# etiiiR/pixel-nerf

Hardware: AMD Instinct MI355X
Metric: rays/sec (coarse+fine, 64+64 samples) (higher is better)
Workload: dtype f32 (f16x3)

## Files before the change

include/pnr_abi.h:

```cpp
#ifndef PNR_ABI_H
#define PNR_ABI_H

#include <stddef.h>
#include <stdint.h>

#ifdef __cplusplus
extern "C" {
#endif

#define PNR_ABI_VERSION 8

typedef enum pnr_status {
    PNR_OK = 0,
    PNR_ERR_INVALID = -1,
    PNR_ERR_UNSUPPORTED = -2,
    PNR_ERR_HIP = -3,
    PNR_ERR_WORKSPACE = -4
} pnr_status;

typedef void *pnr_stream_t;

typedef struct pnr_scene {
    const float *latent;
    const float *cams;
// ... 106 lines not shown

int pnr_point_query_proj(const pnr_scene *scene, const pnr_mlp_desc *desc, const void *packed,
                         const float *proj, const float *xyz, const float *viewdirs,
                         int64_t points_per_obj, float *out, void *workspace,
                         size_t workspace_bytes, pnr_stream_t stream);
int pnr_render_forward_proj(const pnr_scene *scene, const pnr_mlp_desc *desc,
                            const void *coarse_packed, const void *fine_packed,
                            const float *coarse_proj, const float *fine_proj,
                            const pnr_rays *rays, const pnr_rng *rng,
                            const pnr_render_cfg *cfg, const pnr_render_out *out,
                            void *workspace, size_t workspace_bytes, pnr_stream_t stream,
                            void *const *events);

int32_t pnr_render_set_fused(int32_t on);

int pnr_sample_coarse(const float *rays, int64_t n_rays, int32_t n_coarse,
                      const float *u_coarse, int32_t lindisp, float *z,
                      pnr_stream_t stream);

int pnr_sample_fine(const float *rays, int64_t n_rays, int32_t n_coarse,
                    const float *z_coarse, const float *coarse_weights,
                    const float *coarse_depth, int32_t n_fine, int32_t n_fine_depth,
                    float depth_std, const float *u_fine, const float *u_fine_jit,
                    const float *n_depth, int32_t lindisp, float *z_fine,
                    pnr_stream_t stream);

int pnr_composite(const float *z, const float *raw, const float *rays, int64_t n_rays,
                  int32_t k, int32_t white_bkgd, float *weights, float *rgb, float *depth,
                  pnr_stream_t stream);

// ... 109 lines not shown
```

pixel-nerf_amd/csrc/abi.cpp:

```cpp
#include <atomic>
#include <cstdarg>
#include <cstdio>
#include <cstring>

#include "march_dev.h"
#include "pnr_launch.h"

namespace pnr {

static thread_local char g_err[1024];
static std::atomic<int> g_fused_default{2};

void set_error(const char *fmt, ...) {
    va_list ap;
    va_start(ap, fmt);
    vsnprintf(g_err, sizeof(g_err), fmt, ap);
    va_end(ap);
}

int fail(int status, const char *fmt, ...) {
    va_list ap;
    va_start(ap, fmt);
    vsnprintf(g_err, sizeof(g_err), fmt, ap);
    va_end(ap);
// ... 447 lines not shown
                                   nullptr, nullptr, 1, n * kf, raw_new, xsum, st, nullptr, fine_proj)))
            return rc;
        if ((rc = launch_merge_raw(origin, rawc, raw_new, n, kc, kf, rawf, st))) return rc;
    } else if ((rc = launch_point_mlp(*scene, *desc, fine_packed, rays->rays, zf, kall, rays->rays_per_obj,
                                      nullptr, nullptr, 1, n * kall, rawf, xsum, st, nullptr, fine_proj))) {
        return rc;
    }
    if ((rc = mark(5))) return rc;
    if ((rc = launch_composite(zf, rawf, rays->rays, n, kall, cfg->white_bkgd, out->fine_weights,
                               out->fine_rgb, out->fine_depth, st)))
        return rc;
    return mark(6);
}

int32_t pnr_render_set_fused(int32_t on) { return g_fused_default.exchange(on < 0 || on > 3 ? 2 : on); }

int pnr_sample_coarse(const float *rays, int64_t n_rays, int32_t n_coarse, const float *u_coarse,
                      int32_t lindisp, float *z, pnr_stream_t stream) {
    if (n_rays < 0 || n_coarse < 1) return fail(PNR_ERR_INVALID, "pnr_sample_coarse: bad sizes");
    if (n_rays > 0 && (!rays || !u_coarse || !z)) return fail(PNR_ERR_INVALID, "pnr_sample_coarse: NULL");
    return launch_sample_coarse(rays, n_rays, n_coarse, RngSrc{u_coarse, 0, 0, PNR_RNG_U_COARSE}, lindisp, z,
                                (hipStream_t)stream);
}

int pnr_sample_fine(const float *rays, int64_t n_rays, int32_t n_coarse, const float *z_coarse,
                    const float *coarse_weights, const float *coarse_depth, int32_t n_fine,
                    int32_t n_fine_depth, float depth_std, const float *u_fine,
                    const float *u_fine_jit, const float *n_depth, int32_t lindisp, float *z_fine,
                    pnr_stream_t stream) {
    if (n_rays < 0 || n_coarse < 1 || n_fine < 1 || n_fine_depth < 0 || n_fine_depth > n_fine)
// ... 133 lines not shown
```

pixel-nerf_amd/csrc/march_dev.h:

```cpp
#pragma once
#include "pnr_common.h"

namespace pnr {

#ifndef EPI_T
#define EPI_DECL
#define EPI_T(i) ((void)0)
#endif

__device__ __forceinline__ void wave_lds_sync() { asm volatile("s_waitcnt lgkmcnt(0)" ::: "memory"); }

__device__ __forceinline__ float linspace_at(int i, int n, float end, float step) {
    if (n == 1) return 0.0f;
    return (i < n / 2) ? mul_rn(step, (float)i) : sub_rn(end, mul_rn(step, (float)(n - 1 - i)));
}

__device__ __forceinline__ float coarse_z(const RngSrc &u, int64_t b, int kc, int k, float near, float far,
                                          bool lindisp) {
    const float end = (float)(1.0 - 1.0 / (double)kc);
    const float lstep = (kc > 1) ? __fdiv_rn(end, (float)(kc - 1)) : 0.0f;
    const float step = (float)(1.0 / (double)kc);
    const float t = add_rn(linspace_at(k, kc, end, lstep), mul_rn(rng_uniform(u, b, kc, k), step));
    return t_to_z(t, near, far, lindisp);
}

template <int S>
__device__ __forceinline__ float composite_wave(int lane, int64_t b, int K, float far, const float (&zk)[S],
                                                const f4 (&v)[S], int white_bkgd, float *weights,
                                                float *rgb_out, float *depth_out, float (&wk)[S]) {
    double carry = 1.0;
    float sr = 0.f, sg = 0.f, sb = 0.f, sd = 0.f, sw = 0.f;
#pragma unroll
    for (int i = 0; i < S; ++i) {
        const int k = 64 * i + lane;
        const bool valid = k < K;
        const float nxt0 = i + 1 < S ? __int_as_float(__builtin_amdgcn_readlane(__float_as_int(zk[i + 1 < S ? i + 1 : i]), 0))
                                     : far;
        const float zl = dpp_f<0x130>(nxt0, zk[i]);
// ... 217 lines not shown
```

pixel-nerf_amd/csrc/mlp.hip:

```cpp
#include "pnr_diag.h"
#include <cstddef>

#ifdef PNR_EPI_TIMING
__device__ unsigned long long g_epi[8];
#endif

#include "march_dev.h"
#include "mlp_dev.h"
#include "pnr_launch.h"

namespace pnr {
namespace mlpk {

#ifdef PNR_PHASE_TIMING
__device__ unsigned long long g_phase[PT_SLOTS];
#endif

struct Args {
    const float *packed;
    Layout L;
    int render_mode;
    const float *rays, *zs;
    int K;
    int64_t rays_per_obj;
// ... 56 lines not shown
        float *w = scr;
#pragma unroll
        for (int i = 0; i < S; ++i) w[64 * i + lane] = wk[i];
        wave_lds_sync();
        sample_fine_wave(lane, b, near, far, COLS * S, w, buf, depth, kf, c->kfd, c->depth_std, RngSrc{}, RngSrc{},
                         RngSrc{}, c->lindisp != 0, c->n_sort, scr + 128, scr + 256, nullptr, c->z_fine, nullptr,
                         nullptr, true, d, c->single ? const_cast<float *>(buf) : nullptr);
    }
}
__device__ __forceinline__ void march_epilogue(const Args &a, int64_t b, const float *buf, const float *nf,
                                               float *scr, int lane, bool fine_pass) {
    if ((fine_pass ? march_cfg(a)->kpt_f : march_cfg(a)->kpt) == 1) march_ray<1>(a, b, buf, nf, scr, lane, fine_pass);
    else march_ray<2>(a, b, buf, nf, scr, lane, fine_pass);
}

template <int PREC, bool PZ, bool MARCH>
__global__ __launch_bounds__(NTHR) void k_point_mlp(Args a) {
    constexpr int KD = H_DIST;
    constexpr bool HP = is_h(PREC);
    constexpr int NP = nparts(PREC);
    static_assert(PREC != 1 || PZ, "PREC 1 is built for the projected-latent path only");
    extern __shared__ __attribute__((aligned(16))) float smem[];
    constexpr FwdLds M = fwd_lds(HP);
    float *inbuf = smem;
    const int tid = threadIdx.x;
    const int lane = tid & 63;
    const int wave = __builtin_amdgcn_readfirstlane(tid >> 6);
    const int g = lane >> 4;
    const int cl = lane & 15;
    const Layout &L = a.L;

    const int64_t wl_off = (int64_t)(RTW * wave) * 256 + lane * 4;
// ... 29 lines not shown
#ifdef PNR_PHASE_TIMING
    for (int i = 0; i < PT_SLOTS; ++i) gc.pt[i] = 0;
    gc.pt_last = __builtin_amdgcn_s_memtime();
#endif
    constexpr int FPT = 64 / WAVES;

    const int64_t P = a.n_points, PS = P * a.ns;
    float *sv_f = a.save, *sv_z = a.save ? a.save + PS * 64 : nullptr;
    auto sv_slot = [&](int i) { return sv_z + PS * H * (1 + i); };
    uint32_t *sv_mask = a.save ? reinterpret_cast<uint32_t *>(a.save + save_mask_offset(L.n_blocks, PS)) : nullptr;
    auto pre_publish_sync = [&]() {
        if constexpr (!HP)
            lds_barrier();
    };
    auto publish_relu = [&](const Acc &acc, int64_t tile, int save_idx, int64_t row0) {
        if (a.save) {
            save_relu(acc, sv_slot(save_idx) + row0 * H, tile, P, wave, lane);
            save_mask(acc, sv_mask + PS * 16 * save_idx + row0 * 16, tile, P, wave, lane);
        }
        if constexpr (HP) {
            PT(gc, 17);
            relu_colmax(acc, cmax, wave, lane);
            PT(gc, 13);
            lds_barrier();
            PT(gc, 14);
            relu_store_split<true, NP>(acc, P0, P1, cmax, ecol, wave, lane, gc.ecl);
            PT(gc, 15);
        } else {
            store_relu(acc, inbuf, wave, lane);
        }
    };

    Acc x, h;
    int *s_next = reinterpret_cast<int *>(inbuf + M.s_next);
    float *hpart = inbuf + M.hpart;
    float *mreg = inbuf + M.mreg;
    float *mscr = inbuf + M.mscr;
    float *mnf = inbuf + M.mnf;
    const int kpt = MARCH ? march_cfg(a)->kpt : 1;
    const bool single = MARCH && march_cfg(a)->single;
    const int upt = single ? kpt + march_cfg(a)->kpt_f : kpt;
    float *petab_f = inbuf + M.petab_f;
    if (single && wave == 1) petab_f[lane & 31] = march_cfg(a)->packed_f[lane & 31];
    auto grab = [&]() -> int {
        const int64_t T = a.n_tiles / upt;
        const int x0 = blockIdx.x & 7;
        for (int k = 0; k < 8; ++k) {
            const int x = (x0 + k) & 7;
            const int64_t lo = x * T / 8, hi = (x + 1) * T / 8;
            if (lo >= hi) continue;
            const int64_t i = lo + claim_one(a.tile_ctr + 16 * x);
            if (i < hi) return (int)(i * upt);
        }
        return (int)a.n_tiles;
    };
    if (wave == 0) *s_next = grab();
    lds_barrier();
    for (int64_t tile = *s_next; tile < a.n_tiles; tile = *s_next) {
        const int64_t unit = tile / upt;
        const int s_in = (int)(tile - unit * upt);
        const bool pass_f = single && s_in >= kpt;
        const int sub = pass_f ? s_in - kpt : s_in;
        const int kpt_t = pass_f ? march_cfg(a)->kpt_f : kpt;
        auto ray_of = [&]() -> int64_t {
            const int *o = MARCH ? march_cfg(a)->order : nullptr;
            if (!o) return unit;
            const int64_t r = o[unit];
            return r >= 0 && r < a.n_tiles / upt ? r : unit;
        };
        auto PK = [&]() -> const float * { return pass_f ? march_cfg(a)->packed_f : a.packed; };
        auto PJ_ = [&]() -> const float * { return pass_f ? march_cfg(a)->proj_f : a.proj; };
        const float *bias = PK() + L.off_bias;
        gc.hdr = PK();
        auto xp_ptr = [&]() { return a.xsum + (int64_t)blockIdx.x * (2 * COLS * H) + wave * (RTW * CT * 256) + opaque_lane(lane) * 4; };
        auto xs_ptr = [&]() { return xp_ptr() + COLS * H; };

        for (int v = 0; v < a.ns; ++v) {
            const int tid_t = opaque_lane(tid);
            const int col = tid_t / WAVES, qt = tid_t % WAVES;
            const int64_t p_raw = tile * COLS + col;
            const int64_t p = p_raw < a.n_points ? p_raw : a.n_points - 1;
            float px, py, pz, dx, dy, dz, zz = 0.f;
            int64_t obj;
            if (a.render_mode) {
                const int64_t b = MARCH ? ray_of() : p / a.K;
                const int kk = MARCH ? sub * COLS + col : (int)(p - b * a.K);
                const int kt = MARCH ? COLS * kpt_t : a.K;
                const float *ray = a.rays + b * 8;
                if (MARCH && pass_f) {
                    lds_barrier();
                    zz = mreg[kk];
                } else if (MARCH && march_cfg(a)->sample_coarse) {
                    const CfgPtr m = march_cfg(a);
                    zz = coarse_z(ld_rng(m->u_coarse), b, kt, kk, ray[6], ray[7], m->lindisp != 0);
                    float *zo = m->z_out;
                    if (zo && qt == 0 && v == 0) zo[b * kt + kk] = zz;
                } else {
                    zz = a.zs[b * kt + kk];
                }
                dx = ray[3]; dy = ray[4]; dz = ray[5];
                px = add_rn(ray[0], mul_rn(zz, dx));
                py = add_rn(ray[1], mul_rn(zz, dy));
                pz = add_rn(ray[2], mul_rn(zz, dz));
                obj = b / a.rays_per_obj;
            } else {
                px = a.xyz[p * 3 + 0]; py = a.xyz[p * 3 + 1]; pz = a.xyz[p * 3 + 2];
                if (a.dirs) { dx = a.dirs[p * 3 + 0]; dy = a.dirs[p * 3 + 1]; dz = a.dirs[p * 3 + 2]; }
                else { dx = dy = dz = 0.f; }
                obj = p / a.points_per_obj;
            }
            PT_WAIT();
            PT(gc, 8);
            const float *cam = a.cams + (obj * a.ns + v) * 16;
            float xr[3], vd[3], xc[3];
#pragma unroll
            for (int i = 0; i < 3; ++i) {
                const float r0 = cam[3 * i], r1 = cam[3 * i + 1], r2 = cam[3 * i + 2];
                xr[i] = add_rn(add_rn(mul_rn(r0, px), mul_rn(r1, py)), mul_rn(r2, pz));
                vd[i] = add_rn(add_rn(mul_rn(r0, dx), mul_rn(r1, dy)), mul_rn(r2, dz));
                xc[i] = add_rn(xr[i], cam[9 + i]);
            }
            const float fx = cam[12], fy = cam[13], cx = cam[14], cy = cam[15];
            PT_WAIT();
            PT(gc, 9);
            lds_barrier();
            PT(gc, 10);
            if (MARCH && qt == 0 && v == 0) {
                if (!pass_f) mreg[sub * COLS + col] = zz;
                if (col == 0 && sub == 0) {
                    const float *rr = a.rays + ray_of() * 8;
                    mnf[0] = rr[6];
                    mnf[1] = rr[7];
                }
            }
            {
                const int npe = 3 * L.pe_n;
                const float *pet = MARCH && pass_f ? petab_f : petab;
                float fv[FPT];
#pragma unroll
                for (int i = 0; i < FPT; ++i) {
                    const int f = FPT * qt + i;
                    float val = 0.f;
                    if (f < 3) val = xr[f];
                    else if (f < 3 + npe) {
                        const int m = f - 3, q = m / 3, d = m - 3 * q;
                        const float xd = d == 0 ? xr[0] : (d == 1 ? xr[1] : xr[2]);
                        val = sinf(add_rn(pet[16 + q], mul_rn(xd, pet[q])));
                    } else if (f < 6 + npe) {
                        const int d = f - 3 - npe;
                        val = d == 0 ? vd[0] : (d == 1 ? vd[1] : vd[2]);
                    }
                    fv[i] = val;
                }
                if (a.save && p_raw < a.n_points) {
#pragma unroll
                    for (int i = 0; i < FPT / 4; ++i)
                        *reinterpret_cast<f4 *>(sv_f + (v * P + p_raw) * 64 + FPT * qt + 4 * i) =
                            f4{fv[4 * i], fv[4 * i + 1], fv[4 * i + 2], fv[4 * i + 3]};
                }
                if constexpr (HP) {
                    float m = 0.f;
#pragma unroll
                    for (int i = 0; i < FPT; ++i) m = fmaxf(m, fabsf(fv[i]));
#pragma unroll
                    for (int o = 1; o < WAVES; o <<= 1) m = fmaxf(m, __shfl_xor(m, o, 64));
                    const int e = scale_exp(m);
                    const float sc = __builtin_ldexpf(1.f, e);
#pragma unroll
                    for (int i = 0; i < FPT / 4; ++i)
                        put_split4(P0, P1, col * ROWH + swz(col, FPT * qt + 4 * i),
                                   f4{fv[4 * i], fv[4 * i + 1], fv[4 * i + 2], fv[4 * i + 3]}, sc);
                    if (qt == 0) ecol[col] = e;
                } else {
#pragma unroll
                    for (int i = 0; i < FPT / 4; ++i)
                        *reinterpret_cast<f4 *>(inbuf + col * LDS_LD + FPT * qt + 4 * i) =
                            f4{fv[4 * i], fv[4 * i + 1], fv[4 * i + 2], fv[4 * i + 3]};
                }
            }
            PT(gc, 11);
            float u = mul_rn(__fdiv_rn(-xc[0], xc[2]), fx);
            float w = mul_rn(__fdiv_rn(-xc[1], xc[2]), fy);
            u = add_rn(u, cx);
            w = add_rn(w, cy);
            const float wlf = (float)a.wl, hlf = (float)a.hl;
            const float lsx = mul_rn(__fdiv_rn(wlf, sub_rn(wlf, 1.f)), 2.f);
            const float lsy = mul_rn(__fdiv_rn(hlf, sub_rn(hlf, 1.f)), 2.f);
            const float gx = sub_rn(mul_rn(u, __fdiv_rn(lsx, a.img_w)), 1.f);
            const float gy = sub_rn(mul_rn(w, __fdiv_rn(lsy, a.img_h)), 1.f);
            float ix = mul_rn(add_rn(gx, 1.f), mul_rn(sub_rn(wlf, 1.f), 0.5f));
            float iy = mul_rn(add_rn(gy, 1.f), mul_rn(sub_rn(hlf, 1.f), 0.5f));
            ix = fminf(fmaxf(ix, 0.f), wlf - 1.f);
            iy = fminf(fmaxf(iy, 0.f), hlf - 1.f);
            const float x0f = floorf(ix), y0f = floorf(iy);
            const float we = sub_rn(ix, x0f), wn = sub_rn(iy, y0f);
            const float ee = sub_rn(1.f, we), ss = sub_rn(1.f, wn);
            float wnw = mul_rn(ss, ee), wne = mul_rn(ss, we), wsw = mul_rn(wn, ee), wse = mul_rn(wn, we);
            const int x0 = (int)x0f, y0 = (int)y0f;
            const int x1 = x0 + 1 < a.wl ? x0 + 1 : x0, y1 = y0 + 1 < a.hl ? y0 + 1 : y0;
            if (x0 + 1 >= a.wl) { wne = 0.f; wse = 0.f; }
            if (y0 + 1 >= a.hl) { wsw = 0.f; wse = 0.f; }
            if (qt == 0) {
                const uint32_t base = (uint32_t)((obj * a.ns + v) * (int64_t)a.hl * a.wl * H);
                const uint32_t o00 = base + (uint32_t)(y0 * a.wl + x0) * H, o01 = base + (uint32_t)(y0 * a.wl + x1) * H;
                const uint32_t o10 = base + (uint32_t)(y1 * a.wl + x0) * H, o11 = base + (uint32_t)(y1 * a.wl + x1) * H;
                float *t = gtab + col * 8;
                *reinterpret_cast<f4 *>(t) = f4{__uint_as_float(o00), __uint_as_float(o01),
                                                __uint_as_float(o10), __uint_as_float(o11)};
                *reinterpret_cast<f4 *>(t + 4) = f4{wnw, wne, wsw, wse};
            }
            PT(gc, 12);
            lds_barrier();
            PT(gc, 0);
            add_bias(x, bias, wave, lane, false);
            layer_gemm<PREC, NKB_IN, KD, false, 2>(x, PK() + L.off_lin_in, gc, 0);
            for (int blk = 0; blk < L.ncomb; ++blk) {
                const int lz = layer_index(blk, 0, L.ncomb);
                if constexpr (PZ) {
// ... 62 lines not shown
                layer_gemm<PREC, NKB, KD, HP>(h, PK() + L.off_l512 + (int64_t)(lz + 1) * L.layer_floats, gc, 2 + lz,
                                          HP ? &R0 : nullptr);
                pre_publish_sync();
                HRing<KD, NP> R1;
                const float *w1p = PK() + L.off_l512 + (int64_t)(lz + 2) * L.layer_floats;
                if constexpr (HP) hring_prime(R1, w1p + opaque_lane((int)gc.ws_off));
                f4 nb1[RTW];
                load_bias(nb1, bias + (3 + lz) * H, wave, lane);
                publish_relu(h, tile, L.n_blocks + blk, v * P);
                lds_barrier();
                PT(gc, 16);
                set_bias(x, nb1, true);
                layer_gemm<PREC, NKB, KD, HP>(x, PK() + L.off_l512 + (int64_t)(lz + 2) * L.layer_floats, gc, 3 + lz,
                                          HP ? &R1 : nullptr);
            }
            if (a.ns > 1) {
                float *xs = xs_ptr();
                if (v == 0) {
#pragma unroll
                    for (int r = 0; r < RTW; ++r)
#pragma unroll
                        for (int c = 0; c < CT; ++c)
                            *reinterpret_cast<f4 *>(xs + (r * CT + c) * 256) = x[r][c];
                } else if (v < a.ns - 1) {
#pragma unroll
                    for (int r = 0; r < RTW; ++r)
#pragma unroll
                        for (int c = 0; c < CT; ++c) {
                            f4 *ptr = reinterpret_cast<f4 *>(xs + (r * CT + c) * 256);
                            *ptr = *ptr + x[r][c];
                        }
// ... 27 lines not shown
            HRing<KD, NP> R1;
            const float *w1p = PK() + L.off_l512 + (int64_t)(l0 + 1) * L.layer_floats;
            if constexpr (HP) hring_prime(R1, w1p + opaque_lane((int)gc.ws_off));
            f4 nb1[RTW];
            load_bias(nb1, bias + (2 + l0) * H, wave, lane);
            publish_relu(h, tile, L.n_blocks + blk, 0);
            lds_barrier();
            PT(gc, 16);
            set_bias(x, nb1, true);
            layer_gemm<PREC, NKB, KD, HP>(x, PK() + L.off_l512 + (int64_t)(l0 + 1) * L.layer_floats, gc, 2 + l0,
                                      HP ? &R1 : nullptr);
        }
        if (wave == 0) *s_next = s_in + 1 < upt ? (int)tile + 1 : grab();
        pre_publish_sync();
        if constexpr (HP) {
            if (a.save) {
                save_relu(x, sv_slot(2 * L.n_blocks), tile, P, wave, lane);
                save_mask(x, sv_mask + PS * 16 * (2 * L.n_blocks), tile, P, wave, lane);
            }
        } else {
            publish_relu(x, tile, 2 * L.n_blocks, 0);
            lds_barrier();
        }
        PT(gc, 16);
        PT(gc, 3);
        if (HP) {
            const int ln = opaque_lane(lane), g4 = ln >> 4, c16 = ln & 15;
            const float *w32 = PK() + L.off_out32;
            f4 o[CT];
#pragma unroll
            for (int c = 0; c < CT; ++c) o[c] = f4{0.f, 0.f, 0.f, 0.f};
#pragma unroll
            for (int r = 0; r < RTW; ++r) {
// ... 92 lines not shown
    if (reset) {
        static const unsigned long long zero[mlpk::PT_SLOTS] = {};
        if (hipMemcpyToSymbol(HIP_SYMBOL(mlpk::g_phase), zero, sizeof(zero)) != hipSuccess) return -1;
    }
    return 0;
}
#endif
int64_t mlp_save_floats(const pnr_mlp_desc &d, int64_t n_points) {
    return mlpk::save_floats_per_point(d.n_blocks) * n_points;
}

size_t mlp_xsum_bytes(int ns) {
    (void)ns;
    return sizeof(float) * (size_t)device_cu_count() * 2 * mlpk::COLS * mlpk::H + 512;
}

int launch_point_mlp(const pnr_scene &sc, const pnr_mlp_desc &d, const void *packed,
                     const float *rays, const float *zs, int K, int64_t rays_per_obj,
                     const float *xyz, const float *dirs, int64_t points_per_obj,
                     int64_t n_points, float *out, float *xsum_ws, hipStream_t st, float *save,
                     const float *proj, const MarchCfg *march) {
    if (n_points == 0) return PNR_OK;
    if (d.precision == PNR_PREC_F16 && (!proj || save))
        return fail(PNR_ERR_UNSUPPORTED, "precision 1 (f16) is inference only on the projected-latent path: it "
                    "needs the latent projection and takes no activation save; use precision 3 (f16x3)");
    if (proj && save) return fail(PNR_ERR_UNSUPPORTED, "the activation save (training) needs the latent gather path");
    if (march && (!rays || save || (march->kpt != 1 && march->kpt != 2) || K != mlpk::COLS * march->kpt ||
                  n_points % K != 0 || (march->kf > 0 && (K > 64 || march->n_sort > 128 || K + march->kf > march->n_sort))))
        return fail(PNR_ERR_INVALID, "point_mlp: fused march needs K = 64 kpt (kpt 1 or 2) and kc + kf <= 128");
    if (march && march->single &&
// ... 13 lines not shown
    a.ns = sc.n_views; a.hl = sc.latent_h; a.wl = sc.latent_w;
    a.img_w = sc.image_w; a.img_h = sc.image_h;
    a.out = out;
    a.xsum = xsum_ws;
    a.march = march != nullptr;
    if (march) a.m = *march;
    a.n_tiles = (n_points + mlpk::COLS - 1) / mlpk::COLS;
    a.save = save;
    a.proj = proj;
    a.proj_stride = (int64_t)sc.n_obj * sc.n_views * sc.latent_h * sc.latent_w * mlpk::H;
    const int cus = device_cu_count();
    if (a.n_tiles >= (1ll << 31)) return fail(PNR_ERR_UNSUPPORTED, "more than 2^31 point tiles in one launch");
    a.tile_ctr = reinterpret_cast<int *>(xsum_ws + (size_t)cus * 2 * mlpk::COLS * mlpk::H);
    if (hipMemsetAsync(a.tile_ctr, 0, 512, st) != hipSuccess) return fail(PNR_ERR_HIP, "point_mlp: hipMemsetAsync failed");
    const int64_t grid = a.n_tiles < cus ? a.n_tiles : cus;
    const size_t lds = mlpk::lds_bytes(mlpk::fwd_lds(mlpk::is_h(d.precision)), march != nullptr);
#define PNR_LAUNCH_MLP(P)                                                                              \
    do {                                                                                               \
        if (proj && march) hipLaunchKernelGGL((mlpk::k_point_mlp<P, true, true>), dim3((unsigned)grid), dim3(mlpk::NTHR), lds, st, a); \
        else if (proj) hipLaunchKernelGGL((mlpk::k_point_mlp<P, true, false>), dim3((unsigned)grid), dim3(mlpk::NTHR), lds, st, a); \
        else if (march) hipLaunchKernelGGL((mlpk::k_point_mlp<P, false, true>), dim3((unsigned)grid), dim3(mlpk::NTHR), lds, st, a); \
        else hipLaunchKernelGGL((mlpk::k_point_mlp<P, false, false>), dim3((unsigned)grid), dim3(mlpk::NTHR), lds, st, a);     \
    } while (0)
    switch (d.precision) {
    case PNR_PREC_F16:
        if (march) hipLaunchKernelGGL((mlpk::k_point_mlp<1, true, true>), dim3((unsigned)grid), dim3(mlpk::NTHR), lds, st, a);
        else hipLaunchKernelGGL((mlpk::k_point_mlp<1, true, false>), dim3((unsigned)grid), dim3(mlpk::NTHR), lds, st, a);
        break;
    case PNR_PREC_F16X3: PNR_LAUNCH_MLP(3); break;
    case PNR_PREC_BF16X6: PNR_LAUNCH_MLP(6); break;
    case PNR_PREC_BF16X9: PNR_LAUNCH_MLP(9); break;
// ... 8 lines not shown
```

pixel-nerf_amd/csrc/mlp_layout.h:

```cpp
#pragma once
#include "pnr_common.h"

namespace pnr {
namespace mlpk {

constexpr int H = 512;
constexpr int NRT = H / 16;
constexpr int NKB = H / 16;
constexpr int NKB_IN = 4;
constexpr int WAVES = 8;
constexpr int NTHR = 64 * WAVES;
constexpr int RTW = NRT / WAVES;
constexpr int CT = 4;
constexpr int COLS = 16 * CT;
constexpr int LDS_LD = H + 4;
constexpr int KB_FLOATS = NRT * 256;
constexpr int LAYER_FLOATS = NKB * KB_FLOATS;
constexpr int HDR = 64;
constexpr int KS32 = H / 32;
constexpr int KS32_IN = 2;
constexpr int SRT_FLOATS = 768;
constexpr int SKS_FLOATS = NRT * SRT_FLOATS;
constexpr int SRT16_FLOATS = 512;
constexpr int SKS16_FLOATS = NRT * SRT16_FLOATS;
// ... 46 lines not shown

__host__ __device__ constexpr int64_t save_floats_per_point(int n_blocks) {
    return 64 + (int64_t)H * (2 + 2 * n_blocks) + 16 * (2 * n_blocks + 1);
}
__host__ __device__ constexpr int64_t save_mask_offset(int n_blocks, int64_t n_points) {
    return (64 + (int64_t)H * (2 + 2 * n_blocks)) * n_points;
}

__device__ __forceinline__ int scale_exp(float m) {
    if (!(m > 0.f) || !(m < 3.0e38f)) return 0;
    int e = 14 - __builtin_amdgcn_frexp_expf(m);
    return e < -64 ? -64 : (e > 40 ? 40 : e);
}

struct FwdLds {
    int stg, gtab, cmax, ecol, petab, s_next, prog, hpart, mreg, mscr, mnf, petab_f, end;
};
constexpr int IMG_H_FLOATS = PART_HALVES;
constexpr int MARCH_BUF_FLOATS = 640;
constexpr FwdLds fwd_lds(bool hp) {
    FwdLds m = {};
    m.stg = COLS * LDS_LD;
    m.gtab = hp ? IMG_H_FLOATS : m.stg + 2 * STG_FLOATS;
    m.cmax = m.gtab + COLS * 8;
    m.ecol = m.cmax + COLS * 8;
    m.petab = hp ? m.ecol + COLS : m.gtab + COLS * 8;
    m.s_next = m.petab + 32;
    m.prog = m.petab + 40;
    m.hpart = m.petab + 64;
    m.mreg = hp ? m.hpart + WAVES * COLS * 4 : m.petab + 36;
    m.mscr = m.mreg + MARCH_BUF_FLOATS;
    m.mnf = m.mscr + 3 * 128;
    m.petab_f = m.mnf + 4;
    m.end = m.petab_f + 32;
    return m;
}
constexpr size_t lds_bytes(const FwdLds &m, bool march) { return sizeof(float) * (size_t)(march ? m.end : m.mreg); }
constexpr int MARCH_LDS_FLOATS = fwd_lds(true).end - fwd_lds(true).mreg;

struct BwdLds {
    int cmax, ecol, prog, end;
};
constexpr BwdLds bwd_lds() {
    BwdLds m = {};
    m.cmax = IMG_H_FLOATS;
    m.ecol = m.cmax + COLS * 8;
    m.prog = m.ecol + COLS;
    m.end = m.prog + WAVES;
    return m;
}
constexpr size_t lds_bytes(const BwdLds &m) { return sizeof(float) * (size_t)m.end; }

static_assert(lds_bytes(fwd_lds(true), false) == 147968 && lds_bytes(fwd_lds(false), false) == 158864 &&
              lds_bytes(bwd_lds()) == 137504, "LDS totals");
static_assert(lds_bytes(fwd_lds(true), true) == 147968 + 4 * MARCH_LDS_FLOATS &&
              lds_bytes(fwd_lds(false), true) == 158864 + 4 * MARCH_LDS_FLOATS &&
              fwd_lds(false).end - fwd_lds(false).mreg == MARCH_LDS_FLOATS, "LDS totals with the march region");
static_assert(lds_bytes(fwd_lds(true), true) <= 160 * 1024 && lds_bytes(fwd_lds(false), true) <= 160 * 1024 &&
              lds_bytes(bwd_lds()) <= 160 * 1024, "one workgroup's LDS");
static_assert(sizeof(float) * COLS * LDS_LD <= 2 * sizeof(_Float16) * PART_HALVES,
              "the fp32 stage fits in the split image it aliases");

}
}
```

pixel-nerf_amd/csrc/pnr_launch.h:

```cpp
#pragma once
#include "pnr_common.h"

namespace pnr {

struct MarchCfg;

int launch_sample_coarse(const float *, int64_t, int, const RngSrc &, int, float *, hipStream_t);
int launch_sample_fine(const float *, int64_t, int, const float *, const float *, const float *,
                       int, int, float, const RngSrc &, const RngSrc &, const RngSrc &, int, float *,
                       hipStream_t, int *origin = nullptr, float *z_new = nullptr);
int launch_rng_fill(const RngSrc &, int64_t, int, float *, hipStream_t);
int launch_merge_raw(const int *, const float *, const float *, int64_t, int, int, float *, hipStream_t);
int launch_gen_rays(const float *, int64_t, int, int, int, float, float, float, float, float, float,
                    float *, hipStream_t);
int launch_composite(const float *, const float *, const float *, int64_t, int, int, float *,
                     float *, float *, hipStream_t);
int sort_width(int n);
size_t mlp_packed_bytes(const pnr_mlp_desc &);
int mlp_check_desc(const pnr_mlp_desc &);
int mlp_pack(const pnr_mlp_weights &, void *, size_t, hipStream_t);
size_t mlp_packed_t_bytes(const pnr_mlp_desc &);
int mlp_pack_t(const pnr_mlp_weights &, const void *, void *, size_t, hipStream_t);
size_t mlp_xsum_bytes(int ns);
int64_t mlp_save_floats(const pnr_mlp_desc &d, int64_t n_points);
int launch_point_mlp(const pnr_scene &, const pnr_mlp_desc &, const void *, const float *,
                     const float *, int, int64_t, const float *, const float *, int64_t, int64_t,
                     float *, float *, hipStream_t, float *save = nullptr, const float *proj = nullptr,
                     const MarchCfg *march = nullptr);
int launch_mlp_bwd(const pnr_mlp_desc &, const void *, const void *, const float *, const float *, const float *,
                   int64_t, float *, float *, hipStream_t, float *, void *, size_t, int n_views);
size_t mlp_bwd_workspace_bytes(const pnr_mlp_desc &, int64_t);
size_t wgrad_workspace_bytes(int, int64_t);
int launch_wgrad(const float *const *, const float *const *, float *const *, int, int64_t, void *, size_t,
                 hipStream_t, int arith);
int launch_fold_bn(const pnr_bn_fold *, int, int64_t, hipStream_t);
int launch_latent_cl_bwd(const float *, float *const *, const int32_t *, const int32_t *, const int32_t *, int, int, int,
                         int, hipStream_t);
int launch_latent_cl(const float *const *, const int32_t *, const int32_t *, const int32_t *, int, int, float *,
                     int, int, bool, hipStream_t);
int launch_composite_bwd(const float *, const float *, const float *, int64_t, int, int, const float *,
                         const float *, const float *, float *, float *, hipStream_t);
int launch_points_in_bwd(const float *, const float *, int, int64_t, int64_t, int, const float *, const float *,
                         int, int, float, float, const float *, int, const float *, const float *, float *,
// ... 14 lines not shown
```

pixel-nerf_amd/csrc/torch_ops.cpp:

```cpp
#include <ATen/ATen.h>
#include <c10/core/DeviceGuard.h>
#include <c10/hip/HIPStream.h>
#include <torch/library.h>

#include <vector>

#include "../../include/pnr_abi.h"

namespace {

void check(int rc, const char *what) {
    TORCH_CHECK(rc == PNR_OK, what, " failed (status ", rc, "): ", pnr_last_error());
}

void *stream_of(const at::Tensor &t) {
    return c10::hip::getCurrentHIPStream(t.device().index()).stream();
}

const float *fptr(const at::Tensor &t, const char *name) {
    TORCH_CHECK(t.is_cuda(), name, " must be on the HIP device");
    TORCH_CHECK(t.scalar_type() == at::kFloat, name, " must be float32");
    TORCH_CHECK(t.is_contiguous(), name, " must be contiguous");
    return t.data_ptr<float>();
}
// ... 196 lines not shown
    at::Tensor rgb = at::empty({B, 3}, o), depth = at::empty({B}, o);
    check(pnr_composite(fptr(z, "z"), fptr(raw, "raw"), fptr(rays, "rays"), B, (int32_t)K, (int32_t)white_bkgd,
                        want_weights ? w.data_ptr<float>() : nullptr, rgb.data_ptr<float>(), depth.data_ptr<float>(),
                        stream_of(z)),
          "pnr::composite");
    return {w, rgb, depth};
}

std::vector<at::Tensor> composite_meta(const at::Tensor &z, const at::Tensor &raw, const at::Tensor &rays,
                                       bool white_bkgd, bool want_weights) {
    const auto o = f32_like(z);
    return {want_weights ? at::empty({z.size(0), z.size(1)}, o) : at::empty({0}, o), at::empty({z.size(0), 3}, o),
            at::empty({z.size(0)}, o)};
}

}

TORCH_LIBRARY(pnr, m) {
    m.def("render_rays(Tensor latent_cl, Tensor cams, int n_obj, int n_views, float image_w, float image_h, "
          "int[] desc, Tensor coarse_packed, Tensor fine_packed, Tensor? coarse_proj, Tensor? fine_proj, "
          "Tensor rays, int rays_per_obj, int n_coarse, int n_fine, int n_fine_depth, float depth_std, "
          "bool white_bkgd, bool lindisp, Tensor? u_coarse, Tensor? u_fine, Tensor? u_fine_jit, Tensor? n_depth, "
          "int seed, int offset, bool want_weights, bool want_z, int[] events=[], int march_mode=-1, "
          "Tensor? ray_order=None) -> Tensor[]");
    m.def("point_query(Tensor latent_cl, Tensor cams, int n_obj, int n_views, float image_w, float image_h, "
          "int[] desc, Tensor packed, Tensor? proj, Tensor xyz, Tensor? viewdirs) -> Tensor");
    m.def("composite(Tensor z, Tensor raw, Tensor rays, bool white_bkgd, bool want_weights) -> Tensor[]");
}

TORCH_LIBRARY_IMPL(pnr, CUDA, m) {
    m.impl("render_rays", &render_rays);
    m.impl("point_query", &point_query);
    m.impl("composite", &composite);
}

TORCH_LIBRARY_IMPL(pnr, Meta, m) {
    m.impl("render_rays", &render_rays_meta);
    m.impl("point_query", &point_query_meta);
    m.impl("composite", &composite_meta);
}
```

pixel-nerf_amd/pnr/_lib.py:

```python
import ctypes
import os

import torch

_HERE = os.path.dirname(os.path.abspath(__file__))
LIB_PATH = os.environ.get("PNR_LIB_PATH") or os.path.join(_HERE, "libpnr.so")

c_f = ctypes.c_float
c_i32 = ctypes.c_int32
c_i64 = ctypes.c_int64
c_size = ctypes.c_size_t
c_vp = ctypes.c_void_p
PF = ctypes.POINTER(ctypes.c_float)


class Scene(ctypes.Structure):
    _fields_ = [("latent", c_vp), ("cams", c_vp), ("n_obj", c_i32), ("n_views", c_i32),
                ("latent_h", c_i32), ("latent_w", c_i32), ("latent_c", c_i32),
                ("image_w", c_f), ("image_h", c_f)]


class MlpDesc(ctypes.Structure):
    _fields_ = [("d_in", c_i32), ("d_latent", c_i32), ("d_hidden", c_i32), ("d_out", c_i32),
                ("n_blocks", c_i32), ("combine_layer", c_i32), ("pe_n", c_i32),
# ... 49 lines not shown
                                   ctypes.POINTER(RenderCfg), ctypes.POINTER(RenderOut), c_vp,
                                   c_size, c_vp]),
    "pnr_render_forward_events": (c_i32, [ctypes.POINTER(Scene), ctypes.POINTER(MlpDesc), c_vp, c_vp,
                                          ctypes.POINTER(Rays), ctypes.POINTER(Rng),
                                          ctypes.POINTER(RenderCfg), ctypes.POINTER(RenderOut),
                                          c_vp, c_size, c_vp, ctypes.POINTER(c_vp)]),
    "pnr_latent_project_bytes": (c_size, [ctypes.POINTER(Scene), ctypes.POINTER(MlpDesc)]),
    "pnr_latent_project": (c_i32, [ctypes.POINTER(Scene), ctypes.POINTER(MlpWeights), c_vp, c_size, c_vp]),
    "pnr_point_query_proj": (c_i32, [ctypes.POINTER(Scene), ctypes.POINTER(MlpDesc), c_vp, c_vp, c_vp, c_vp,
                                     c_i64, c_vp, c_vp, c_size, c_vp]),
    "pnr_render_forward_proj": (c_i32, [ctypes.POINTER(Scene), ctypes.POINTER(MlpDesc), c_vp, c_vp, c_vp, c_vp,
                                        ctypes.POINTER(Rays), ctypes.POINTER(Rng),
                                        ctypes.POINTER(RenderCfg), ctypes.POINTER(RenderOut),
                                        c_vp, c_size, c_vp, ctypes.POINTER(c_vp)]),
    "pnr_render_set_fused": (c_i32, [c_i32]),
    "pnr_sample_coarse": (c_i32, [c_vp, c_i64, c_i32, c_vp, c_i32, c_vp, c_vp]),
    "pnr_sample_fine": (c_i32, [c_vp, c_i64, c_i32, c_vp, c_vp, c_vp, c_i32, c_i32, c_f, c_vp,
                                c_vp, c_vp, c_i32, c_vp, c_vp]),
    "pnr_composite": (c_i32, [c_vp, c_vp, c_vp, c_i64, c_i32, c_i32, c_vp, c_vp, c_vp, c_vp]),
    "pnr_rng_fill": (c_i32, [ctypes.c_uint64, ctypes.c_uint64, c_i32, c_i64, c_i32, c_vp, c_vp]),
    "pnr_gen_rays": (c_i32, [c_vp, c_i64, c_i32, c_i32, c_i32, c_f, c_f, c_f, c_f, c_f, c_f, c_vp, c_vp]),
    "pnr_latent_channels_last": (c_i32, [ctypes.POINTER(c_vp), ctypes.POINTER(c_i32), ctypes.POINTER(c_i32),
                                         ctypes.POINTER(c_i32), c_i32, c_i32, c_vp, c_i32, c_i32, c_vp]),
    "pnr_latent_channels_last_nhwc": (c_i32, [ctypes.POINTER(c_vp), ctypes.POINTER(c_i32), ctypes.POINTER(c_i32),
                                              ctypes.POINTER(c_i32), c_i32, c_i32, c_vp, c_i32, c_i32, c_vp]),
    "pnr_fold_batchnorm": (c_i32, [c_vp, c_i32, c_i64, c_vp]),
    "pnr_latent_channels_last_backward": (c_i32, [c_vp, c_vp, c_vp, c_vp, c_vp, c_i32, c_i32, c_i32, c_i32, c_vp]),
    "pnr_point_save_floats": (c_size, [ctypes.POINTER(MlpDesc), c_i64]),
    "pnr_render_points": (c_i32, [ctypes.POINTER(Scene), ctypes.POINTER(MlpDesc), c_vp,
                                  ctypes.POINTER(Rays), c_vp, c_i32, c_vp, c_vp, c_vp, c_size, c_vp]),
# ... 71 lines not shown

class fused_march:

    def __init__(self, mode):
        self.on = int(mode)

    def __enter__(self):
        self.prev = load().pnr_render_set_fused(self.on)
        return self

    def __exit__(self, *exc):
        load().pnr_render_set_fused(self.prev)
        return False


def stream_of(device):
    return ctypes.c_void_p(torch.cuda.current_stream(device).cuda_stream)
```

Measured before the change: 449,500.

## Add lean specialization of fused-march MLP kernel for single-view fp16 render

```diff
diff --git a/include/pnr_abi.h b/include/pnr_abi.h
--- a/include/pnr_abi.h
+++ b/include/pnr_abi.h
@@ -144,6 +144,12 @@
 
 int32_t pnr_render_set_fused(int32_t on);
 
+#define PNR_MLP_KERNEL_NONE 0
+#define PNR_MLP_KERNEL_GENERAL 1
+#define PNR_MLP_KERNEL_LEAN 2
+int32_t pnr_mlp_set_lean(int32_t on);
+int32_t pnr_mlp_last_kernel(void);
+
 int pnr_sample_coarse(const float *rays, int64_t n_rays, int32_t n_coarse,
                       const float *u_coarse, int32_t lindisp, float *z,
                       pnr_stream_t stream);
diff --git a/pixel-nerf_amd/csrc/abi.cpp b/pixel-nerf_amd/csrc/abi.cpp
--- a/pixel-nerf_amd/csrc/abi.cpp
+++ b/pixel-nerf_amd/csrc/abi.cpp
@@ -485,6 +485,8 @@
 }
 
 int32_t pnr_render_set_fused(int32_t on) { return g_fused_default.exchange(on < 0 || on > 3 ? 2 : on); }
+int32_t pnr_mlp_set_lean(int32_t on) { return pnr::mlp_set_lean(on); }
+int32_t pnr_mlp_last_kernel(void) { return pnr::mlp_last_kernel(); }
 
 int pnr_sample_coarse(const float *rays, int64_t n_rays, int32_t n_coarse, const float *u_coarse,
                       int32_t lindisp, float *z, pnr_stream_t stream) {
diff --git a/pixel-nerf_amd/csrc/march_dev.h b/pixel-nerf_amd/csrc/march_dev.h
--- a/pixel-nerf_amd/csrc/march_dev.h
+++ b/pixel-nerf_amd/csrc/march_dev.h
@@ -15,13 +15,24 @@
     return (i < n / 2) ? mul_rn(step, (float)i) : sub_rn(end, mul_rn(step, (float)(n - 1 - i)));
 }
 
+struct CoarseSteps {
+    float end, lstep, step;
+};
+__device__ __forceinline__ CoarseSteps coarse_steps(int kc) {
+    CoarseSteps s;
+    s.end = (float)(1.0 - 1.0 / (double)kc);
+    s.lstep = (kc > 1) ? __fdiv_rn(s.end, (float)(kc - 1)) : 0.0f;
+    s.step = (float)(1.0 / (double)kc);
+    return s;
+}
+__device__ __forceinline__ float coarse_z_at(const RngSrc &u, int64_t b, int kc, int k, float near, float far,
+                                             bool lindisp, const CoarseSteps &s) {
+    const float t = add_rn(linspace_at(k, kc, s.end, s.lstep), mul_rn(rng_uniform(u, b, kc, k), s.step));
+    return t_to_z(t, near, far, lindisp);
+}
 __device__ __forceinline__ float coarse_z(const RngSrc &u, int64_t b, int kc, int k, float near, float far,
                                           bool lindisp) {
-    const float end = (float)(1.0 - 1.0 / (double)kc);
-    const float lstep = (kc > 1) ? __fdiv_rn(end, (float)(kc - 1)) : 0.0f;
-    const float step = (float)(1.0 / (double)kc);
-    const float t = add_rn(linspace_at(k, kc, end, lstep), mul_rn(rng_uniform(u, b, kc, k), step));
-    return t_to_z(t, near, far, lindisp);
+    return coarse_z_at(u, b, kc, k, near, far, lindisp, coarse_steps(kc));
 }
 
 template <int S>
diff --git a/pixel-nerf_amd/csrc/mlp.hip b/pixel-nerf_amd/csrc/mlp.hip
--- a/pixel-nerf_amd/csrc/mlp.hip
+++ b/pixel-nerf_amd/csrc/mlp.hip
@@ -1,4 +1,5 @@
 #include "pnr_diag.h"
+#include <atomic>
 #include <cstddef>
 
 #ifdef PNR_EPI_TIMING
@@ -94,8 +95,14 @@
     else march_ray<2>(a, b, buf, nf, scr, lane, fine_pass);
 }
 
-template <int PREC, bool PZ, bool MARCH>
+typedef const __attribute__((address_space(4))) float *CFloatPtr;
+typedef const __attribute__((address_space(4))) int *CIntPtr;
+__device__ __forceinline__ CFloatPtr as_const(const float *p) { return (CFloatPtr)(uint64_t)p; }
+__device__ __forceinline__ CIntPtr as_const(const int *p) { return (CIntPtr)(uint64_t)p; }
+
+template <int PREC, bool PZ, bool MARCH, bool LEAN = false>
 __global__ __launch_bounds__(NTHR) void k_point_mlp(Args a) {
+    static_assert(!LEAN || (PZ && MARCH && is_h(PREC)), "LEAN is the fused-march render on the projected latent");
     constexpr int KD = H_DIST;
     constexpr bool HP = is_h(PREC);
     constexpr int NP = nparts(PREC);
@@ -155,9 +162,11 @@
             lds_barrier();
     };
     auto publish_relu = [&](const Acc &acc, int64_t tile, int save_idx, int64_t row0) {
-        if (a.save) {
-            save_relu(acc, sv_slot(save_idx) + row0 * H, tile, P, wave, lane);
-            save_mask(acc, sv_mask + PS * 16 * save_idx + row0 * 16, tile, P, wave, lane);
+        if constexpr (!LEAN) {
+            if (a.save) {
+                save_relu(acc, sv_slot(save_idx) + row0 * H, tile, P, wave, lane);
+                save_mask(acc, sv_mask + PS * 16 * save_idx + row0 * 16, tile, P, wave, lane);
+            }
         }
         if constexpr (HP) {
             PT(gc, 17);
@@ -179,10 +188,36 @@
     float *mscr = inbuf + M.mscr;
     float *mnf = inbuf + M.mnf;
     const int kpt = MARCH ? march_cfg(a)->kpt : 1;
-    const bool single = MARCH && march_cfg(a)->single;
+    const bool single = !LEAN && MARCH && march_cfg(a)->single;
     const int upt = single ? kpt + march_cfg(a)->kpt_f : kpt;
     float *petab_f = inbuf + M.petab_f;
     if (single && wave == 1) petab_f[lane & 31] = march_cfg(a)->packed_f[lane & 31];
+    struct ProjK {
+        float wlf, hlf, kx, ky, hx, hy;
+    };
+    auto proj_consts = [&]() -> ProjK {
+        const float wlf = (float)a.wl, hlf = (float)a.hl;
+        const float lsx = mul_rn(__fdiv_rn(wlf, sub_rn(wlf, 1.f)), 2.f);
+        const float lsy = mul_rn(__fdiv_rn(hlf, sub_rn(hlf, 1.f)), 2.f);
+        return ProjK{wlf, hlf, __fdiv_rn(lsx, a.img_w), __fdiv_rn(lsy, a.img_h), mul_rn(sub_rn(wlf, 1.f), 0.5f),
+                     mul_rn(sub_rn(hlf, 1.f), 0.5f)};
+    };
+    float *ltab = inbuf + M.ltab;
+    if constexpr (LEAN) {
+        const CoarseSteps cs = coarse_steps(COLS * kpt);
+        const ProjK pk = proj_consts();
+        if (wave == 0) {
+            ltab[LT_END] = cs.end;
+            ltab[LT_LSTEP] = cs.lstep;
+            ltab[LT_STEP] = cs.step;
+            ltab[LT_WLF] = pk.wlf;
+            ltab[LT_HLF] = pk.hlf;
+            ltab[LT_KX] = pk.kx;
+            ltab[LT_KY] = pk.ky;
+            ltab[LT_HX] = pk.hx;
+            ltab[LT_HY] = pk.hy;
+        }
+    }
     auto grab = [&]() -> int {
         const int64_t T = a.n_tiles / upt;
         const int x0 = blockIdx.x & 7;
@@ -197,8 +232,13 @@
     };
     if (wave == 0) *s_next = grab();
     lds_barrier();
-    for (int64_t tile = *s_next; tile < a.n_tiles; tile = *s_next) {
-        const int64_t unit = tile / upt;
+    auto take = [&]() -> int64_t {
+        const int t = *s_next;
+        if constexpr (LEAN) return __builtin_amdgcn_readfirstlane(t);
+        else return t;
+    };
+    for (int64_t tile = take(); tile < a.n_tiles; tile = take()) {
+        const int64_t unit = LEAN ? (upt == 2 ? tile >> 1 : tile) : tile / upt;
         const int s_in = (int)(tile - unit * upt);
         const bool pass_f = single && s_in >= kpt;
         const int sub = pass_f ? s_in - kpt : s_in;
@@ -206,8 +246,14 @@
         auto ray_of = [&]() -> int64_t {
             const int *o = MARCH ? march_cfg(a)->order : nullptr;
             if (!o) return unit;
-            const int64_t r = o[unit];
-            return r >= 0 && r < a.n_tiles / upt ? r : unit;
+            if constexpr (LEAN) {
+                const int r = as_const(o)[unit];
+                const int n_units = upt == 2 ? (int)a.n_tiles >> 1 : (int)a.n_tiles;
+                return r >= 0 && r < n_units ? (int64_t)r : unit;
+            } else {
+                const int64_t r = o[unit];
+                return r >= 0 && r < a.n_tiles / upt ? r : unit;
+            }
         };
         auto PK = [&]() -> const float * { return pass_f ? march_cfg(a)->packed_f : a.packed; };
         auto PJ_ = [&]() -> const float * { return pass_f ? march_cfg(a)->proj_f : a.proj; };
@@ -216,14 +262,48 @@
         auto xp_ptr = [&]() { return a.xsum + (int64_t)blockIdx.x * (2 * COLS * H) + wave * (RTW * CT * 256) + opaque_lane(lane) * 4; };
         auto xs_ptr = [&]() { return xp_ptr() + COLS * H; };
 
-        for (int v = 0; v < a.ns; ++v) {
+        auto NS = [&]() -> int {
+            if constexpr (LEAN) return 1;
+            else return a.ns;
+        };
+        for (int v = 0; v < NS(); ++v) {
             const int tid_t = opaque_lane(tid);
             const int col = tid_t / WAVES, qt = tid_t % WAVES;
             const int64_t p_raw = tile * COLS + col;
             const int64_t p = p_raw < a.n_points ? p_raw : a.n_points - 1;
             float px, py, pz, dx, dy, dz, zz = 0.f;
             int64_t obj;
-            if (a.render_mode) {
+            float cam_s[16], nf_s[2];
+            if constexpr (LEAN) {
+                const int64_t b = ray_of();
+                const int kk = sub * COLS + col;
+                const int kt = COLS * kpt_t;
+                const CFloatPtr rp = as_const(a.rays) + b * 8;
+                float ray[8];
+#pragma unroll
+                for (int i = 0; i < 8; ++i) ray[i] = rp[i];
+                int64_t rpo = a.rays_per_obj;
+                asm volatile("" : "+s"(rpo));
+                obj = b < rpo ? 0 : b / rpo;
+                const CFloatPtr cp = as_const(a.cams) + obj * 16;
+#pragma unroll
+                for (int i = 0; i < 16; ++i) cam_s[i] = cp[i];
+                if (march_cfg(a)->sample_coarse) {
+                    const CfgPtr m = march_cfg(a);
+                    const CoarseSteps cs = {ltab[LT_END], ltab[LT_LSTEP], ltab[LT_STEP]};
+                    zz = coarse_z_at(ld_rng(m->u_coarse), b, kt, kk, ray[6], ray[7], m->lindisp != 0, cs);
+                    float *zo = m->z_out;
+                    if (zo && qt == 0) zo[b * kt + kk] = zz;
+                } else {
+                    zz = a.zs[b * kt + kk];
+                }
+                dx = ray[3]; dy = ray[4]; dz = ray[5];
+                px = add_rn(ray[0], mul_rn(zz, dx));
+                py = add_rn(ray[1], mul_rn(zz, dy));
+                pz = add_rn(ray[2], mul_rn(zz, dz));
+                nf_s[0] = ray[6];
+                nf_s[1] = ray[7];
+            } else if (a.render_mode) {
                 const int64_t b = MARCH ? ray_of() : p / a.K;
                 const int kk = MARCH ? sub * COLS + col : (int)(p - b * a.K);
                 const int kt = MARCH ? COLS * kpt_t : a.K;
@@ -252,16 +332,20 @@
             }
             PT_WAIT();
             PT(gc, 8);
-            const float *cam = a.cams + (obj * a.ns + v) * 16;
+            const float *cam_p = a.cams + (obj * NS() + v) * 16;
+            auto cam = [&](int i) -> float {
+                if constexpr (LEAN) return cam_s[i];
+                else return cam_p[i];
+            };
             float xr[3], vd[3], xc[3];
 #pragma unroll
             for (int i = 0; i < 3; ++i) {
-                const float r0 = cam[3 * i], r1 = cam[3 * i + 1], r2 = cam[3 * i + 2];
+                const float r0 = cam(3 * i), r1 = cam(3 * i + 1), r2 = cam(3 * i + 2);
                 xr[i] = add_rn(add_rn(mul_rn(r0, px), mul_rn(r1, py)), mul_rn(r2, pz));
                 vd[i] = add_rn(add_rn(mul_rn(r0, dx), mul_rn(r1, dy)), mul_rn(r2, dz));
-                xc[i] = add_rn(xr[i], cam[9 + i]);
-            }
-            const float fx = cam[12], fy = cam[13], cx = cam[14], cy = cam[15];
+                xc[i] = add_rn(xr[i], cam(9 + i));
+            }
+            const float fx = cam(12), fy = cam(13), cx = cam(14), cy = cam(15);
             PT_WAIT();
             PT(gc, 9);
             lds_barrier();
@@ -269,9 +353,14 @@
             if (MARCH && qt == 0 && v == 0) {
                 if (!pass_f) mreg[sub * COLS + col] = zz;
                 if (col == 0 && sub == 0) {
-                    const float *rr = a.rays + ray_of() * 8;
-                    mnf[0] = rr[6];
-                    mnf[1] = rr[7];
+                    if constexpr (LEAN) {
+                        mnf[0] = nf_s[0];
+                        mnf[1] = nf_s[1];
+                    } else {
+                        const float *rr = a.rays + ray_of() * 8;
+                        mnf[0] = rr[6];
+                        mnf[1] = rr[7];
+                    }
                 }
             }
             {
@@ -293,11 +382,13 @@
                     }
                     fv[i] = val;
                 }
-                if (a.save && p_raw < a.n_points) {
-#pragma unroll
-                    for (int i = 0; i < FPT / 4; ++i)
-                        *reinterpret_cast<f4 *>(sv_f + (v * P + p_raw) * 64 + FPT * qt + 4 * i) =
-                            f4{fv[4 * i], fv[4 * i + 1], fv[4 * i + 2], fv[4 * i + 3]};
+                if constexpr (!LEAN) {
+                    if (a.save && p_raw < a.n_points) {
+#pragma unroll
+                        for (int i = 0; i < FPT / 4; ++i)
+                            *reinterpret_cast<f4 *>(sv_f + (v * P + p_raw) * 64 + FPT * qt + 4 * i) =
+                                f4{fv[4 * i], fv[4 * i + 1], fv[4 * i + 2], fv[4 * i + 3]};
+                    }
                 }
                 if constexpr (HP) {
                     float m = 0.f;
@@ -324,13 +415,19 @@
             float w = mul_rn(__fdiv_rn(-xc[1], xc[2]), fy);
             u = add_rn(u, cx);
             w = add_rn(w, cy);
-            const float wlf = (float)a.wl, hlf = (float)a.hl;
-            const float lsx = mul_rn(__fdiv_rn(wlf, sub_rn(wlf, 1.f)), 2.f);
-            const float lsy = mul_rn(__fdiv_rn(hlf, sub_rn(hlf, 1.f)), 2.f);
-            const float gx = sub_rn(mul_rn(u, __fdiv_rn(lsx, a.img_w)), 1.f);
-            const float gy = sub_rn(mul_rn(w, __fdiv_rn(lsy, a.img_h)), 1.f);
-            float ix = mul_rn(add_rn(gx, 1.f), mul_rn(sub_rn(wlf, 1.f), 0.5f));
-            float iy = mul_rn(add_rn(gy, 1.f), mul_rn(sub_rn(hlf, 1.f), 0.5f));
+            const ProjK pk = [&]() {
+                if constexpr (LEAN) {
+                    const f4 t = *reinterpret_cast<const f4 *>(ltab + LT_WLF);
+                    return ProjK{t.x, t.y, t.z, t.w, ltab[LT_HX], ltab[LT_HY]};
+                } else {
+                    return proj_consts();
+                }
+            }();
+            const float wlf = pk.wlf, hlf = pk.hlf;
+            const float gx = sub_rn(mul_rn(u, pk.kx), 1.f);
+            const float gy = sub_rn(mul_rn(w, pk.ky), 1.f);
+            float ix = mul_rn(add_rn(gx, 1.f), pk.hx);
+            float iy = mul_rn(add_rn(gy, 1.f), pk.hy);
             ix = fminf(fmaxf(ix, 0.f), wlf - 1.f);
             iy = fminf(fmaxf(iy, 0.f), hlf - 1.f);
             const float x0f = floorf(ix), y0f = floorf(iy);
@@ -342,7 +439,7 @@
             if (x0 + 1 >= a.wl) { wne = 0.f; wse = 0.f; }
             if (y0 + 1 >= a.hl) { wsw = 0.f; wse = 0.f; }
             if (qt == 0) {
-                const uint32_t base = (uint32_t)((obj * a.ns + v) * (int64_t)a.hl * a.wl * H);
+                const uint32_t base = (uint32_t)((obj * NS() + v) * (int64_t)a.hl * a.wl * H);
                 const uint32_t o00 = base + (uint32_t)(y0 * a.wl + x0) * H, o01 = base + (uint32_t)(y0 * a.wl + x1) * H;
                 const uint32_t o10 = base + (uint32_t)(y1 * a.wl + x0) * H, o11 = base + (uint32_t)(y1 * a.wl + x1) * H;
                 float *t = gtab + col * 8;
@@ -435,7 +532,7 @@
                 layer_gemm<PREC, NKB, KD, HP>(x, PK() + L.off_l512 + (int64_t)(lz + 2) * L.layer_floats, gc, 3 + lz,
                                           HP ? &R1 : nullptr);
             }
-            if (a.ns > 1) {
+            if constexpr (!LEAN) if (a.ns > 1) {
                 float *xs = xs_ptr();
                 if (v == 0) {
 #pragma unroll
@@ -493,9 +590,11 @@
         if (wave == 0) *s_next = s_in + 1 < upt ? (int)tile + 1 : grab();
         pre_publish_sync();
         if constexpr (HP) {
-            if (a.save) {
-                save_relu(x, sv_slot(2 * L.n_blocks), tile, P, wave, lane);
-                save_mask(x, sv_mask + PS * 16 * (2 * L.n_blocks), tile, P, wave, lane);
+            if constexpr (!LEAN) {
+                if (a.save) {
+                    save_relu(x, sv_slot(2 * L.n_blocks), tile, P, wave, lane);
+                    save_mask(x, sv_mask + PS * 16 * (2 * L.n_blocks), tile, P, wave, lane);
+                }
             }
         } else {
             publish_relu(x, tile, 2 * L.n_blocks, 0);
@@ -618,6 +717,11 @@
     (void)ns;
     return sizeof(float) * (size_t)device_cu_count() * 2 * mlpk::COLS * mlpk::H + 512;
 }
+
+static std::atomic<int> g_mlp_lean{1};
+static std::atomic<int> g_mlp_last_kernel{PNR_MLP_KERNEL_NONE};
+int mlp_set_lean(int on) { return g_mlp_lean.exchange(on != 0); }
+int mlp_last_kernel() { return g_mlp_last_kernel.load(std::memory_order_relaxed); }
 
 int launch_point_mlp(const pnr_scene &sc, const pnr_mlp_desc &d, const void *packed,
                      const float *rays, const float *zs, int K, int64_t rays_per_obj,
@@ -661,7 +765,18 @@
     a.tile_ctr = reinterpret_cast<int *>(xsum_ws + (size_t)cus * 2 * mlpk::COLS * mlpk::H);
     if (hipMemsetAsync(a.tile_ctr, 0, 512, st) != hipSuccess) return fail(PNR_ERR_HIP, "point_mlp: hipMemsetAsync failed");
     const int64_t grid = a.n_tiles < cus ? a.n_tiles : cus;
-    const size_t lds = mlpk::lds_bytes(mlpk::fwd_lds(mlpk::is_h(d.precision)), march != nullptr);
+    size_t lds = mlpk::lds_bytes(mlpk::fwd_lds(mlpk::is_h(d.precision)), march != nullptr);
+    const bool lean = g_mlp_lean.load(std::memory_order_relaxed) && mlpk::is_h(d.precision) && proj && march &&
+                      !march->single && rays && sc.n_views == 1 && !save;
+    g_mlp_last_kernel.store(lean ? PNR_MLP_KERNEL_LEAN : PNR_MLP_KERNEL_GENERAL, std::memory_order_relaxed);
+    if (lean) {
+        lds = mlpk::lds_bytes_lean(mlpk::fwd_lds(true));
+        if (d.precision == PNR_PREC_F16)
+            hipLaunchKernelGGL((mlpk::k_point_mlp<1, true, true, true>), dim3((unsigned)grid), dim3(mlpk::NTHR), lds, st, a);
+        else
+            hipLaunchKernelGGL((mlpk::k_point_mlp<3, true, true, true>), dim3((unsigned)grid), dim3(mlpk::NTHR), lds, st, a);
+        return launch_ok("point_mlp") ? PNR_OK : PNR_ERR_HIP;
+    }
 #define PNR_LAUNCH_MLP(P)                                                                              \
     do {                                                                                               \
         if (proj && march) hipLaunchKernelGGL((mlpk::k_point_mlp<P, true, true>), dim3((unsigned)grid), dim3(mlpk::NTHR), lds, st, a); \
diff --git a/pixel-nerf_amd/csrc/mlp_layout.h b/pixel-nerf_amd/csrc/mlp_layout.h
--- a/pixel-nerf_amd/csrc/mlp_layout.h
+++ b/pixel-nerf_amd/csrc/mlp_layout.h
@@ -84,8 +84,9 @@
 }
 
 struct FwdLds {
-    int stg, gtab, cmax, ecol, petab, s_next, prog, hpart, mreg, mscr, mnf, petab_f, end;
+    int stg, gtab, cmax, ecol, petab, s_next, prog, hpart, mreg, mscr, mnf, petab_f, end, ltab;
 };
+enum LeanTab { LT_END = 0, LT_LSTEP, LT_STEP, LT_PAD, LT_WLF, LT_HLF, LT_KX, LT_KY, LT_HX, LT_HY, LT_FLOATS = 16 };
 constexpr int IMG_H_FLOATS = PART_HALVES;
 constexpr int MARCH_BUF_FLOATS = 640;
 constexpr FwdLds fwd_lds(bool hp) {
@@ -103,9 +104,11 @@
     m.mnf = m.mscr + 3 * 128;
     m.petab_f = m.mnf + 4;
     m.end = m.petab_f + 32;
+    m.ltab = m.end;
     return m;
 }
 constexpr size_t lds_bytes(const FwdLds &m, bool march) { return sizeof(float) * (size_t)(march ? m.end : m.mreg); }
+constexpr size_t lds_bytes_lean(const FwdLds &m) { return sizeof(float) * (size_t)(m.ltab + LT_FLOATS); }
 constexpr int MARCH_LDS_FLOATS = fwd_lds(true).end - fwd_lds(true).mreg;
 
 struct BwdLds {
@@ -128,6 +131,9 @@
               fwd_lds(false).end - fwd_lds(false).mreg == MARCH_LDS_FLOATS, "LDS totals with the march region");
 static_assert(lds_bytes(fwd_lds(true), true) <= 160 * 1024 && lds_bytes(fwd_lds(false), true) <= 160 * 1024 &&
               lds_bytes(bwd_lds()) <= 160 * 1024, "one workgroup's LDS");
+static_assert(lds_bytes_lean(fwd_lds(true)) == lds_bytes(fwd_lds(true), true) + 4 * LT_FLOATS &&
+              lds_bytes_lean(fwd_lds(true)) <= 160 * 1024 && fwd_lds(true).ltab % 4 == 0,
+              "the lean table fits beside the fp16 map and the march region, 16-byte aligned");
 static_assert(sizeof(float) * COLS * LDS_LD <= 2 * sizeof(_Float16) * PART_HALVES,
               "the fp32 stage fits in the split image it aliases");
 
diff --git a/pixel-nerf_amd/csrc/pnr_launch.h b/pixel-nerf_amd/csrc/pnr_launch.h
--- a/pixel-nerf_amd/csrc/pnr_launch.h
+++ b/pixel-nerf_amd/csrc/pnr_launch.h
@@ -27,6 +27,8 @@
                      const float *, int, int64_t, const float *, const float *, int64_t, int64_t,
                      float *, float *, hipStream_t, float *save = nullptr, const float *proj = nullptr,
                      const MarchCfg *march = nullptr);
+int mlp_set_lean(int on);
+int mlp_last_kernel();
 int launch_mlp_bwd(const pnr_mlp_desc &, const void *, const void *, const float *, const float *, const float *,
                    int64_t, float *, float *, hipStream_t, float *, void *, size_t, int n_views);
 size_t mlp_bwd_workspace_bytes(const pnr_mlp_desc &, int64_t);
diff --git a/pixel-nerf_amd/csrc/torch_ops.cpp b/pixel-nerf_amd/csrc/torch_ops.cpp
--- a/pixel-nerf_amd/csrc/torch_ops.cpp
+++ b/pixel-nerf_amd/csrc/torch_ops.cpp
@@ -234,6 +234,9 @@
             at::empty({z.size(0)}, o)};
 }
 
+int64_t mlp_set_lean(bool on) { return pnr_mlp_set_lean(on ? 1 : 0); }
+int64_t mlp_last_kernel() { return pnr_mlp_last_kernel(); }
+
 }
 
 TORCH_LIBRARY(pnr, m) {
@@ -246,6 +249,8 @@
     m.def("point_query(Tensor latent_cl, Tensor cams, int n_obj, int n_views, float image_w, float image_h, "
           "int[] desc, Tensor packed, Tensor? proj, Tensor xyz, Tensor? viewdirs) -> Tensor");
     m.def("composite(Tensor z, Tensor raw, Tensor rays, bool white_bkgd, bool want_weights) -> Tensor[]");
+    m.def("mlp_set_lean(bool on) -> int", &mlp_set_lean);
+    m.def("mlp_last_kernel() -> int", &mlp_last_kernel);
 }
 
 TORCH_LIBRARY_IMPL(pnr, CUDA, m) {
diff --git a/pixel-nerf_amd/pnr/_lib.py b/pixel-nerf_amd/pnr/_lib.py
--- a/pixel-nerf_amd/pnr/_lib.py
+++ b/pixel-nerf_amd/pnr/_lib.py
@@ -87,6 +87,8 @@
                                         ctypes.POINTER(RenderCfg), ctypes.POINTER(RenderOut),
                                         c_vp, c_size, c_vp, ctypes.POINTER(c_vp)]),
     "pnr_render_set_fused": (c_i32, [c_i32]),
+    "pnr_mlp_set_lean": (c_i32, [c_i32]),
+    "pnr_mlp_last_kernel": (c_i32, []),
     "pnr_sample_coarse": (c_i32, [c_vp, c_i64, c_i32, c_vp, c_i32, c_vp, c_vp]),
     "pnr_sample_fine": (c_i32, [c_vp, c_i64, c_i32, c_vp, c_vp, c_vp, c_i32, c_i32, c_f, c_vp,
                                 c_vp, c_vp, c_i32, c_vp, c_vp]),
@@ -188,5 +190,22 @@
         return False
 
 
+MLP_KERNEL_NONE, MLP_KERNEL_GENERAL, MLP_KERNEL_LEAN = 0, 1, 2
+
+
+class lean_mlp:
+
+    def __init__(self, on):
+        self.on = int(bool(on))
+
+    def __enter__(self):
+        self.prev = load().pnr_mlp_set_lean(self.on)
+        return self
+
+    def __exit__(self, *exc):
+        load().pnr_mlp_set_lean(self.prev)
+        return False
+
+
 def stream_of(device):
     return ctypes.c_void_p(torch.cuda.current_stream(device).cuda_stream)
```

Result: faster. 454,400 (median of 6 runs) (+1.1%).
